# LouisPwr/CarpeDeam

Measured on AMD Instinct MI355X. Metric: corrected bases/sec on 50M×100bp synthetic reads (dhigh), 1/2/4/8 GPU, higher is better.
Workload: dtype u8 (2-bit packed bases; int32 scores; software x87 f80 likelihood sums)

## Files before the change

carpedeam_amd/csrc/bucket.h:

```cpp
#pragma once
#include <algorithm>
#include <cstdio>
#include <cstdlib>
#include <cstring>
#include <vector>

#include "common.h"
#include "radix.h"
#include "scan.h"

namespace bucket {

constexpr int BK_NT = 256;
constexpr int BK_WAVES = BK_NT / 64;
constexpr int WV_OWN = 256;
constexpr int WV_WIN = 768;
constexpr int WV_WORDS = WV_WIN / 64;
constexpr int WV_FIRST = 512;
constexpr int BK_GROUP = 256;
constexpr int BK_MAXB = 512;
constexpr int BK_ORD = 8;

__device__ __forceinline__ void waveLdsSync() {
    __builtin_amdgcn_fence(__ATOMIC_RELEASE, "wavefront");
    __builtin_amdgcn_wave_barrier();
    __builtin_amdgcn_fence(__ATOMIC_ACQUIRE, "wavefront");
}

template <int WIN> struct WaveLdsT {
    unsigned long long bits[WIN / 64];
    uint16_t ord[WIN];
};
typedef WaveLdsT<WV_WIN> WaveLds;
template <typename WL> __device__ __forceinline__ int firstSetFrom(const WL &w, int from, int limit) {
    for (int word = from >> 6; word * 64 < limit; word++) {
        unsigned long long m = w.bits[word];
        if (word == (from >> 6)) m &= ~0ull << (from & 63);
        if (m) { const int p = word * 64 + __ffsll(m) - 1; return p < limit ? p : -1; }
    }
    return -1;
}
template <typename WL> __device__ __forceinline__ int lastSetIn(const WL &w, int lo, int hi) {
    const int wl = (lo + 1) >> 6;
    for (int word = hi >> 6; word >= wl; word--) {
        unsigned long long m = w.bits[word];
        if (word == (hi >> 6)) m &= (2ull << (hi & 63)) - 1ull;
        if (word == wl) m &= ~0ull << ((lo + 1) & 63);
        if (m) return word * 64 + 63 - __clzll(m);
    }
    return -1;
}

struct BigList {
    unsigned long long *list;
    unsigned int *cnt;
    __device__ __forceinline__ void add(uint64_t s, uint64_t e) const { if (!list) return; const unsigned int q = atomicAdd(cnt, 1u); list[2 * (size_t) q] = s; list[2 * (size_t) q + 1] = e; }
};

template <int M> __device__ __forceinline__ uint32_t xorLane32(uint32_t a) {
    static_assert(M == 1 || M == 2 || M == 4 || M == 8 || M == 16 || M == 32, "lane distance");
    if (M == 1) return (uint32_t) __builtin_amdgcn_update_dpp(0, (int) a, 0xB1, 0xF, 0xF, false);
    if (M == 2) return (uint32_t) __builtin_amdgcn_update_dpp(0, (int) a, 0x4E, 0xF, 0xF, false);
    if (M == 4) {
        const int t = __builtin_amdgcn_update_dpp(0, (int) a, 0x104, 0xF, 0x5, false);
        return (uint32_t) __builtin_amdgcn_update_dpp(t, (int) a, 0x114, 0xF, 0xA, false);
    }
    if (M == 8) return (uint32_t) __builtin_amdgcn_update_dpp(0, (int) a, 0x128, 0xF, 0xF, false);
    if (M == 16) return (uint32_t) __builtin_amdgcn_ds_swizzle((int) a, 0x401F);
    return (uint32_t) __shfl_xor((int) a, 32, 64);
}
template <typename W, int M> struct XorLane;
template <int M> struct XorLane<uint32_t, M> { __device__ static __forceinline__ uint32_t get(uint32_t a) { return xorLane32<M>(a); } };
template <int M> struct XorLane<uint64_t, M> {
    __device__ static __forceinline__ uint64_t get(uint64_t a) { return ((uint64_t) xorLane32<M>((uint32_t) (a >> 32)) << 32) | xorLane32<M>((uint32_t) a); }
};
typedef unsigned __int128 u128;
template <int M> struct XorLane<u128, M> {
    __device__ static __forceinline__ u128 get(u128 a) { return ((u128) XorLane<uint64_t, M>::get((uint64_t) (a >> 64)) << 64) | XorLane<uint64_t, M>::get((uint64_t) a); }
};
template <typename W> __device__ __forceinline__ W xorLane(W a, int d) {
    switch (d) {
        case 1: return XorLane<W, 1>::get(a);
        case 2: return XorLane<W, 2>::get(a);
        case 4: return XorLane<W, 4>::get(a);
        case 8: return XorLane<W, 8>::get(a);
        case 16: return XorLane<W, 16>::get(a);
        default: return XorLane<W, 32>::get(a);
    }
}
template <typename W> __device__ __forceinline__ W shflUpW(W a, int d);
template <> __device__ __forceinline__ uint32_t shflUpW<uint32_t>(uint32_t a, int d) { return (uint32_t) __shfl_up((int) a, d, 64); }
template <> __device__ __forceinline__ uint64_t shflUpW<uint64_t>(uint64_t a, int d) {
    return ((uint64_t) (uint32_t) __shfl_up((int) (a >> 32), d, 64) << 32) | (uint32_t) __shfl_up((int) (uint32_t) a, d, 64);
}

template <int R, typename W>
__device__ __forceinline__ void bitonicRegs(W (&v)[R], int lane) {
#pragma unroll
    for (int k = 2; k <= 64 * R; k <<= 1) {
#pragma unroll
        for (int j = k >> 1; j > 0; j >>= 1) {
            if (j < R) {
#pragma unroll
                for (int r = 0; r < R; r++) {
                    const int p = r ^ j;
                    if (p > r) {
                        const bool up = (((lane * R + r) & k) == 0);
                        const W a = v[r], b = v[p];
                        const bool sw = (b < a) == up;
                        v[r] = sw ? b : a; v[p] = sw ? a : b;
                    }
                }
            } else {
                const bool lower = ((lane & (j / R)) == 0);
#pragma unroll
                for (int r = 0; r < R; r++) {
                    const bool up = (((lane * R + r) & k) == 0);
                    const W a = v[r], b = xorLane<W>(a, j / R);
                    v[r] = ((b < a) == (up == lower)) ? b : a;
                }
            }
        }
    }
}
template <int R, typename W, typename MakeComp, typename Done>
__device__ __forceinline__ void sortGroupRegs(int gm, int lane, const MakeComp &mk, const Done &done) {
    W v[R];
#pragma unroll
    for (int r = 0; r < R; r++) { const int i = lane * R + r; v[r] = (i < gm) ? mk(i) : (W) ~(W) 0; }
    bitonicRegs<R, W>(v, lane);
    done(v);
}
template <typename W, int MAXR = 8, typename MakeComp, typename Done>
__device__ __forceinline__ void sortGroup(int gm, int lane, const MakeComp &mk, const Done &done) {
    static_assert(MAXR == 1 || MAXR == 2 || MAXR == 4 || MAXR == 8, "networks of 64, 128, 256 and 512 words");
    if (MAXR == 1 || gm <= 64) sortGroupRegs<1, W>(gm, lane, mk, done);
    else if constexpr (MAXR >= 2) {
        if (MAXR == 2 || gm <= 128) sortGroupRegs<2, W>(gm, lane, mk, done);
        else if constexpr (MAXR >= 4) {
            if (MAXR == 4 || gm <= 256) sortGroupRegs<4, W>(gm, lane, mk, done);
            else if constexpr (MAXR >= 8) sortGroupRegs<8, W>(gm, lane, mk, done);
        }
    }
}
__device__ __forceinline__ uint64_t prevLane64(uint64_t a) {
    const uint32_t lo = (uint32_t) __builtin_amdgcn_update_dpp((int) (uint32_t) a, (int) (uint32_t) a, 0x138, 0xF, 0xF, false);
    const uint32_t hi = (uint32_t) __builtin_amdgcn_update_dpp((int) (uint32_t) (a >> 32), (int) (uint32_t) (a >> 32), 0x138, 0xF, 0xF, false);
    return ((uint64_t) hi << 32) | lo;
}
__device__ __forceinline__ uint64_t readLane64(uint64_t a, int l) {
    return ((uint64_t) (uint32_t) __builtin_amdgcn_readlane((int) (uint32_t) (a >> 32), l) << 32) | (uint32_t) __builtin_amdgcn_readlane((int) (uint32_t) a, l);
}

template <typename T, int WIN = WV_WIN, int FIRST = WV_FIRST, int GROUP = BK_GROUP, typename Fetch, typename Put, typename KeyAt, typename GroupFn>
__device__ __forceinline__ void waveBuckets(uint64_t r0, uint64_t n, int own, uint32_t maxBucket, uint64_t hiMask, const BigList &big, WaveLdsT<WIN> &w, int lane,
                                            const Fetch &fetch, const Put &put, const KeyAt &keyAt, const GroupFn &groupFn) {
    constexpr int WV_WIN = WIN, WV_FIRST = FIRST, WV_WORDS = WIN / 64;
    const int avail = (int) min((uint64_t) WV_WIN, n - r0);
    uint64_t carry = r0 ? keyAt(r0 - 1) : 0ull;
    int ordBase = -1;
    auto loadRows = [&](auto rowsTag, int t0, auto fullTag) {
        constexpr int ROWS = decltype(rowsTag)::value;
        constexpr bool FULL = decltype(fullTag)::value;
        T tup[ROWS];
#pragma unroll
        for (int t = 0; t < ROWS; t++) { const int i = (t0 + t) * 64 + lane; if (FULL || i < avail) tup[t] = fetch(r0 + (uint64_t) i); }
#pragma unroll
        for (int t = 0; t < ROWS; t++) {
            const int i = (t0 + t) * 64 + lane;
            const bool valid = FULL || i < avail;
            const uint64_t k = valid ? put(i, tup[t]) : 0ull;
            const bool differs = ((k ^ prevLane64(k)) & hiMask) != 0ull;
            unsigned long long m = __ballot(valid && differs) & ~1ull;
            if ((FULL || (t0 + t) * 64 < avail) && ((r0 == 0 && t0 + t == 0) || ((readLane64(k, 0) ^ carry) & hiMask) != 0ull)) m |= 1ull;
            if (lane == 0) w.bits[t0 + t] = m;
            const int below = (int) __builtin_amdgcn_mbcnt_hi((uint32_t) (m >> 32), __builtin_amdgcn_mbcnt_lo((uint32_t) m, 0u));
            if (valid) w.ord[i] = (uint16_t) (ordBase + below + (int) ((m >> lane) & 1ull));
            ordBase += __popcll(m);
            carry = readLane64(k, 63);
        }
    };
    if (lane >= WV_FIRST / 64 && lane < WV_WORDS) w.bits[lane] = 0ull;
    if (avail >= WV_FIRST) loadRows(std::integral_constant<int, WV_FIRST / 64>(), 0, std::true_type());
    else loadRows(std::integral_constant<int, WV_FIRST / 64>(), 0, std::false_type());
    waveLdsSync();
    const int ownEnd = min(own, avail);
    const int sLast = lastSetIn(w, -1, ownEnd - 1);
    if (sLast < 0) return;
    const int p0 = firstSetFrom(w, 0, ownEnd);
    int loaded = min(avail, WV_FIRST);
    int eLast = firstSetFrom(w, sLast + 1, loaded);
    if constexpr (WV_FIRST < WV_WIN) if (eLast < 0 && loaded < avail) {
        loadRows(std::integral_constant<int, WV_WORDS - WV_FIRST / 64>(), WV_FIRST / 64, std::false_type());
        waveLdsSync();
        loaded = avail;
        eLast = firstSetFrom(w, sLast + 1, loaded);
    }
    if (eLast < 0 && r0 + (uint64_t) avail == n) eLast = avail;
    int eOwn = eLast;
    if (eLast < 0) {
        const uint64_t h = keyAt(r0 + (uint64_t) sLast) & hiMask;
        uint64_t lo = r0 + (uint64_t) avail, hi = n;
        while (lo < hi) { const uint64_t mid = lo + ((hi - lo) >> 1); if ((keyAt(mid) & hiMask) == h) lo = mid + 1; else hi = mid; }
        if (lane == 0) big.add(r0 + (uint64_t) sLast, lo);
        eOwn = sLast;
    }
    int g0 = p0;
    while (g0 < eOwn) {
        const int lim = min(g0 + min(GROUP, (int) maxBucket), eOwn);
        int e = (lim == eOwn) ? eOwn : lastSetIn(w, g0, lim);
        if (e < 0) { e = firstSetFrom(w, g0 + 1, eOwn); if (e < 0) e = eOwn; }
        const int gm = e - g0;
        if (gm > (int) maxBucket) { if (lane == 0) big.add(r0 + (uint64_t) g0, r0 + (uint64_t) e); }
        else groupFn(g0, gm);
        g0 = e;
    }
}

constexpr int WV_IDX = 10;

struct SortArgs {
    const uint64_t *in; uint64_t *out; uint64_t n;
    int shiftHi;
    int ign;
    int own; uint32_t maxBucket;
    BigList big;
};

__global__ __launch_bounds__(BK_NT) void k_bucket_sort(SortArgs a) {
    __shared__ uint64_t sKeyAll[BK_WAVES][WV_WIN];
    __shared__ WaveLds wAll[BK_WAVES];
    const int lane = threadIdx.x & 63, wave = threadIdx.x >> 6;
    const uint64_t r0 = ((uint64_t) blockIdx.x * BK_WAVES + wave) * (uint64_t) a.own;
    if (r0 >= a.n) return;
    uint64_t *sKey = sKeyAll[wave];
    WaveLds &w = wAll[wave];
    const uint64_t lowMask = (1ull << a.shiftHi) - 1ull;
    const int lowW = a.shiftHi - a.ign, ign = a.ign;
    waveBuckets<uint64_t>(r0, a.n, a.own, a.maxBucket, ~lowMask, a.big, w, lane,
        [&](uint64_t g) { return a.in[g]; },
        [&](int i, uint64_t k) { sKey[i] = k; return k; },
        [&](uint64_t g) { return a.in[g]; },
        [&](int g0, int gm) {
            sortGroup<uint64_t>(gm, lane,
                [&](int i) {
                    const uint64_t low = (sKey[g0 + i] & lowMask) >> ign;
                    return ((((uint64_t) w.ord[g0 + i] << lowW) | low) << WV_IDX) | (uint64_t) (g0 + i);
                },
                [&](auto &v) {
                    constexpr int R = sizeof(v) / sizeof(v[0]);
#pragma unroll
                    for (int r = 0; r < R; r++) { const int p = lane * R + r; if (p < gm) a.out[r0 + (uint64_t) (g0 + p)] = sKey[(int) (v[r] & ((1u << WV_IDX) - 1u))]; }
                });
        });
}

template <int WAVES, typename W>
__device__ __forceinline__ void bitonicBlock(W (&v)[8], int lane, int wave, W *sX) {
    constexpr int R = 8, N = 64 * R * WAVES;
    const int base = wave * 64 * R + lane * R;
#pragma unroll
    for (int k = 2; k <= N; k <<= 1) {
#pragma unroll
        for (int j = k >> 1; j > 0; j >>= 1) {
            if (j >= 64 * R) {
                const int pw = wave ^ (j / (64 * R));
#pragma unroll
                for (int r = 0; r < R; r++) sX[(r * WAVES + wave) * 64 + lane] = v[r];
                __syncthreads();
                const bool lower = ((base & j) == 0);
#pragma unroll
                for (int r = 0; r < R; r++) {
                    const bool up = (((base + r) & k) == 0);
                    const W a = v[r], b = sX[(r * WAVES + pw) * 64 + lane];
                    v[r] = ((b < a) == (up == lower)) ? b : a;
                }
                __syncthreads();
            } else if (j >= R) {
                const bool lower = ((lane & (j / R)) == 0);
#pragma unroll
                for (int r = 0; r < R; r++) {
                    const bool up = (((base + r) & k) == 0);
                    const W a = v[r], b = xorLane<W>(a, j / R);
// ... 141 lines not shown
```

carpedeam_amd/csrc/kmer_group.h:

```cpp
#pragma once
#include "kmer_tuple.h"
#include "runsort.h"

namespace {

struct GroupParams {
    uint64_t n;
    int onlyExtendable, covMode; float covThr;
    uint32_t idBits, diagBits; int diagBias;
    int wide;
    uint64_t first;
    uint64_t firstRunIdx;
    unsigned long long *stat;
};
constexpr int STAT_STRIPES = 4096;
__device__ __forceinline__ void waveGroupStats(unsigned long long *stat, uint32_t cnt) {
    if ((threadIdx.x & 63) == 0 && cnt) atomicAdd(stat + ((blockIdx.x * 4 + (threadIdx.x >> 6)) & (STAT_STRIPES - 1)), (unsigned long long) cnt);
}
template <typename LY> struct GroupArgs : GroupParams {
    const uint64_t *keys; const typename LY::V *vals;
    TupleGeom geom;
};
__device__ __forceinline__ bool canBeCoveredK(float covThr, int covMode, float ql, float tl) {
    switch (covMode) {
        case 0: return ((ql / tl >= covThr) && (tl / ql >= covThr));
        case 2: return ((tl / ql) >= covThr);
        case 1: return ((ql / tl) >= covThr);
        case 3: return ((tl / ql) >= covThr) && (tl / ql) <= 1.0;
        case 4: return ((ql / tl) >= covThr) && (ql / tl) <= 1.0;
        case 5: return (fminf(tl, ql) / fmaxf(tl, ql)) >= covThr;
        default: return true;
    }
}
__device__ __forceinline__ uint64_t packGroupKey(const GroupParams &a, uint32_t rep, uint32_t id, int diag, bool noRev) {
    const uint64_t hi = a.wide ? (uint64_t) id : (((uint64_t) rep << a.idBits) | id);
    return (hi << (a.diagBits + 1)) | ((uint64_t) (uint32_t) (diag + a.diagBias) << 1) | (noRev ? 1ull : 0ull);
}
__device__ __forceinline__ uint64_t markRunStart(const GroupParams &a, uint64_t gk, uint32_t rep) {
    return (runsort::gkKept(gk) ? gk : (runsort::GK_DROPPED | ((uint64_t) rep << (a.diagBits + 1)))) | runsort::GK_START;
}
template <typename LY> struct StartIndex {
    const uint64_t *keys; TupleGeom geom; unsigned long long first;
    __device__ unsigned long long operator()(unsigned long long i) const {
        if (i == first) return i;
        const uint64_t a = keys[i], b = keys[i - 1];
        const bool start = (a == ~0ull) || (b == ~0ull) || (LY::kmerOf(a, i, geom) != LY::kmerOf(b, i - 1, geom));
        return start ? i : 0ull;
    }
};
template <typename LY> struct StartFrom {
    StartIndex<LY> f;
    __device__ __forceinline__ unsigned long long operator()(size_t i) const { return f(f.first + (unsigned long long) i); }
};

__device__ __forceinline__ uint64_t groupKeyCore(const GroupParams &a, uint32_t repId, int queryLen, int repPos, bool repIsReverse,
                                                 uint32_t id, int tLen, int tPos0, bool targetIsReverse) {
    int qPos, tPos; bool qRev;
    if (repIsReverse && !targetIsReverse) { qPos = repPos; tPos = tPos0; qRev = true; }
    else if (repIsReverse && targetIsReverse) { qPos = (queryLen - 1) - repPos; tPos = (tLen - 1) - tPos0; qRev = false; }
    else if (!repIsReverse && targetIsReverse) { qPos = (queryLen - 1) - repPos; tPos = (tLen - 1) - tPos0; qRev = true; }
    else { qPos = repPos; tPos = tPos0; qRev = false; }
    const int diagonal = qPos - tPos;
    const bool canBeExtended = diagonal < 0 || (diagonal > (queryLen - tLen));
    const bool cbc = (a.covThr <= 0.0f && a.covMode <= 2 && queryLen > 0 && tLen > 0) ? true : canBeCoveredK(a.covThr, a.covMode, (float) queryLen, (float) tLen);
    const bool keep = (a.onlyExtendable == 0 && cbc) || (canBeExtended && a.onlyExtendable != 0);
    return keep ? packGroupKey(a, repId, id, diagonal, !qRev) : ~0ull;
}
template <typename LY>
__device__ __forceinline__ uint64_t groupKeyOf(const GroupParams &a, const TupleGeom &geom, uint64_t repKey, typename LY::V repVal, uint64_t repSlot, uint32_t repPos0,
                                               bool firstRun, uint64_t key, typename LY::V v, uint64_t slot) {
    return groupKeyCore(a, LY::seqOf(repVal), (int) LY::lenOf(repKey, repVal, repSlot, geom), (int) repPos0, firstRun ? false : ((repKey & BIT63) == 0),
                        LY::seqOf(v), (int) LY::lenOf(key, v, slot, geom), (int) LY::posOf(key, v, slot, geom), (key & BIT63) == 0);
}

template <typename LY>
__global__ __launch_bounds__(256) void k_groups(GroupArgs<LY> a, unsigned long long *__restrict__ startIo ) {
    const uint64_t i = a.first + (uint64_t) blockIdx.x * blockDim.x + threadIdx.x;
    unsigned long long gk = ~0ull;
    if (i < a.n) {
        const uint64_t key = a.keys[i];
        if (key != ~0ull) {
            const uint64_t st = startIo[i];
            const uint64_t km = LY::kmerOf(key, i, a.geom);
            const bool hasNext = (i + 1 < a.n) && a.keys[i + 1] != ~0ull && LY::kmerOf(a.keys[i + 1], i + 1, a.geom) == km;
            if (st != i || hasNext) {
                uint64_t bestKey = a.keys[st]; const typename LY::V best = a.vals[st];
                const uint32_t repId = LY::seqOf(best);
                uint32_t bestPos = LY::posOf(bestKey, best, st, a.geom);
                for (uint64_t e = st + 1; e < a.n && a.keys[e] != ~0ull && LY::kmerOf(a.keys[e], e, a.geom) == km && LY::seqOf(a.vals[e]) == repId; e++) {
                    const uint32_t pe = LY::posOf(a.keys[e], a.vals[e], e, a.geom);
                    if (pe < bestPos) { bestPos = pe; bestKey = a.keys[e]; }
                }
                gk = groupKeyOf<LY>(a, a.geom, bestKey, best, st, bestPos, st == a.firstRunIdx, key, a.vals[i], i);
                if (a.wide && st == i) gk = markRunStart(a, gk, repId);
            }
        }
        startIo[i] = gk;
    }
    waveGroupStats(a.stat, (uint32_t) __popcll(__ballot(runsort::gkKept(gk))));
}

struct BlockHead { int32_t lo, hi; uint32_t td, pad; };
#ifndef CDM_REC_CAP
#define CDM_REC_CAP 32
#endif
constexpr int REC_CAP = CDM_REC_CAP;
static_assert(REC_CAP <= 64, "a wave writes its stage out with one lane per record");
__global__ void k_block_heads(TupleGeom geom, uint64_t n, uint64_t perBlock, uint64_t blocks, BlockHead *__restrict__ out) {
    const uint64_t b = (uint64_t) blockIdx.x * blockDim.x + threadIdx.x;
    if (b >= blocks) return;
    const uint64_t base = b * perBlock;
    const uint32_t td = headDigit(geom, base);
    const uint64_t since = base - geom.seg[td], until = geom.seg[td + 1] - base;
    BlockHead h; h.td = td; h.pad = 0; h.lo = -(int32_t) min(since, (uint64_t) 1 << 30); h.hi = (int32_t) min(until, (uint64_t) 1 << 30);
    out[b] = h;
}
constexpr int REC_WAVES = 256, REC_BIG_LDS = 256;
struct RecCount { const uint8_t *c; __device__ __forceinline__ unsigned long long operator()(size_t i) const { return c[i]; } };
__device__ __forceinline__ uint64_t lowerBoundStart(const uint64_t *__restrict__ val, uint64_t n, uint64_t start) {
    uint64_t lo = 0, hi = n;
    while (lo < hi) { const uint64_t mid = lo + ((hi - lo) >> 1); if ((val[mid] >> runsort::RUN_CNT_BITS) < start) lo = mid + 1; else hi = mid; }
    return lo;
}
__global__ __launch_bounds__(256) void k_rec_compact(const uint32_t *__restrict__ stRep, const uint64_t *__restrict__ stVal, const unsigned long long *__restrict__ off, uint64_t waves,
                                                     uint64_t own, const uint64_t *__restrict__ bigVal, uint64_t nBig, uint32_t *__restrict__ recRep, uint64_t *__restrict__ recVal) {
    __shared__ unsigned long long sOff[REC_WAVES + 1];
    __shared__ uint64_t sBig[REC_BIG_LDS];
    __shared__ uint64_t sB[2];
    const uint64_t w0 = (uint64_t) blockIdx.x * REC_WAVES;
    const int nw = (int) min((uint64_t) REC_WAVES, waves - w0);
    for (int i = threadIdx.x; i <= nw; i += 256) sOff[i] = off[w0 + i];
    if (threadIdx.x < 2) sB[threadIdx.x] = nBig ? lowerBoundStart(bigVal, nBig, (w0 + (threadIdx.x ? (uint64_t) nw : 0ull)) * own) : 0ull;
    __syncthreads();
    const uint64_t b0 = sB[0], nb = sB[1] - sB[0];
    for (uint64_t i = threadIdx.x; i < nb && i < (uint64_t) REC_BIG_LDS; i += 256) sBig[i] = bigVal[b0 + i] >> runsort::RUN_CNT_BITS;
    __syncthreads();
    const unsigned long long base = sOff[0], total = sOff[nw] - base;
    for (unsigned long long i = threadIdx.x; i < total; i += 256) {
        int w = 0;
#pragma unroll
        for (int st = REC_WAVES / 2; st > 0; st >>= 1) if (w + st < nw && sOff[w + st] - base <= i) w += st;
        const uint64_t src = (w0 + (uint64_t) w) * REC_CAP + (i - (sOff[w] - base));
        const uint64_t v = stVal[src], start = v >> runsort::RUN_CNT_BITS;
        uint64_t before = b0;
        if (nb <= (uint64_t) REC_BIG_LDS) { for (uint64_t q = 0; q < nb; q++) before += sBig[q] < start; }
        else before = lowerBoundStart(bigVal, nBig, start);
        recRep[base + i + before] = stRep[src]; recVal[base + i + before] = v;
    }
}
__global__ __launch_bounds__(256) void k_rec_place_big(const uint32_t *__restrict__ bigRep, const uint64_t *__restrict__ bigVal, uint64_t nBig, const uint64_t *__restrict__ stVal,
                                                       const uint8_t *__restrict__ stCnt, const unsigned long long *__restrict__ off, uint64_t own, uint32_t *__restrict__ recRep, uint64_t *__restrict__ recVal) {
    const uint64_t b = (uint64_t) blockIdx.x * blockDim.x + threadIdx.x;
    if (b >= nBig) return;
    const uint64_t v = bigVal[b], start = v >> runsort::RUN_CNT_BITS, w = start / own;
    uint64_t before = off[w];
    const int c = stCnt[w];
    for (int j = 0; j < c; j++) before += (stVal[w * REC_CAP + j] >> runsort::RUN_CNT_BITS) < start;
    recRep[b + before] = bigRep[b]; recVal[b + before] = v;
}
__global__ __launch_bounds__(256) void k_big_gap_copy(const unsigned long long *__restrict__ ranges, unsigned int cnt, const unsigned long long *__restrict__ dense, unsigned long long *__restrict__ gapped) {
    const unsigned int lane = threadIdx.x & 63, wavesPerGrid = gridDim.x * 4;
    for (unsigned int r = blockIdx.x * 4 + (threadIdx.x >> 6); r < cnt; r += wavesPerGrid) {
        const unsigned long long len = ranges[3 * (size_t) r + 1] - ranges[3 * (size_t) r], o = ranges[3 * (size_t) r + 2];
        for (unsigned long long i = lane; i < len; i += 64) gapped[o + r + i] = dense[o + i];
        if (lane == 0) gapped[o + r + len] = ~0ull;
    }
}
__global__ __launch_bounds__(256) void k_big_rec_starts(const unsigned long long *__restrict__ ranges, unsigned int cnt, uint64_t *__restrict__ recVal, uint64_t nRec) {
    const uint64_t j = (uint64_t) blockIdx.x * blockDim.x + threadIdx.x;
    if (j >= nRec) return;
    const uint64_t v = recVal[j], x = v >> runsort::RUN_CNT_BITS;
    unsigned int lo = 0, hi = cnt;
    while (hi - lo > 1) { const unsigned int mid = lo + ((hi - lo) >> 1); if (ranges[3 * (size_t) mid + 2] + mid <= x) lo = mid; else hi = mid; }
    const uint64_t slot = ranges[3 * (size_t) lo] + (x - (ranges[3 * (size_t) lo + 2] + lo));
    recVal[j] = (slot << runsort::RUN_CNT_BITS) | (v & ((1ull << runsort::RUN_CNT_BITS) - 1ull));
}
template <typename LY, typename W>
struct BucketGroupArgs : GroupParams {
    const BlockHead *blockHead = nullptr;
    uint32_t *recRep = nullptr; uint64_t *recVal = nullptr; uint8_t *recCnt = nullptr;
    uint32_t recLimit = REC_CAP;
    uint32_t *ovRep = nullptr; uint64_t *ovVal = nullptr; unsigned long long *ovCursor = nullptr; unsigned long long ovCap = 0;
    const uint64_t *keys; const typename LY::V *vals; TupleGeom geom;
    unsigned long long *out;
    int lowBits;
    int own; uint32_t maxBucket; bucket::BigList big;
};
#ifndef CDM_GK_OWN
#define CDM_GK_OWN 128
#define CDM_GK_WIN 384
#define CDM_GK_FIRST 256
#endif
#ifndef CDM_GKS_OWN
#define CDM_GKS_OWN 256
#define CDM_GKS_WIN 512
#define CDM_GKS_FIRST 384
#endif
#ifndef CDM_GKS_GROUP
#define CDM_GKS_GROUP 256
#endif
template <typename LY> struct GkGeom {
    static constexpr int OWN = LY::bySlot ? CDM_GKS_OWN : CDM_GK_OWN, WIN = LY::bySlot ? CDM_GKS_WIN : CDM_GK_WIN, FIRST = LY::bySlot ? CDM_GKS_FIRST : CDM_GK_FIRST, MAXB = WIN - OWN;
    static constexpr int GROUP = LY::bySlot ? CDM_GKS_GROUP : bucket::BK_GROUP, CAP = MAXB, MAXR = LY::bySlot ? CAP / 64 : 8;
    static_assert(WIN % 64 == 0 && FIRST % 64 == 0 && FIRST <= WIN && OWN <= FIRST && WIN <= (1 << bucket::WV_IDX) && (MAXB == 64 || MAXB == 128 || MAXB == 256 || MAXB == 512), "grouping kernel geometry");
    static_assert(GROUP >= 64 && GROUP <= MAXB && GROUP <= (1 << bucket::BK_ORD), "grouping kernel group capacity");
};
#ifndef CDM_GK_MINW
#define CDM_GK_MINW 0
#endif
template <typename LY> constexpr size_t gkLdsBytes() {
    return (size_t) bucket::BK_WAVES * ((size_t) GkGeom<LY>::WIN * 8 + (LY::bySlot ? 1 : (size_t) GkGeom<LY>::WIN) * sizeof(typename LY::V) + (size_t) GkGeom<LY>::CAP * 4 + sizeof(bucket::WaveLdsT<GkGeom<LY>::WIN>) +
                                      (LY::bySlot ? (size_t) REC_CAP : 1) * 12);
}
template <typename LY> constexpr int gkMinWaves() {
    return LY::bySlot ? (CDM_GK_MINW ? CDM_GK_MINW : 6) : (CDM_GK_MINW ? (int) std::min<size_t>(CDM_GK_MINW, CU_LDS_BYTES / gkLdsBytes<LY>()) : 1);
}
template <typename LY, typename W>
__global__ __launch_bounds__(bucket::BK_NT, gkMinWaves<LY>()) void k_bucket_groups(BucketGroupArgs<LY, W> a) {
    static_assert(bucket::BK_NT == 256 && (size_t) gkMinWaves<LY>() * gkLdsBytes<LY>() <= CU_LDS_BYTES, "the launch bound asks for more blocks per CU than the kernel's LDS lets run: the compiler would drop the request");
    using namespace bucket;
    typedef typename LY::V V;
    constexpr int GK_WIN = GkGeom<LY>::WIN, GK_FIRST = GkGeom<LY>::FIRST, GK_CAP = GkGeom<LY>::CAP;
    __shared__ uint64_t sKeyAll[BK_WAVES][GK_WIN];
    __shared__ V sValAll[BK_WAVES][LY::bySlot ? 1 : GK_WIN];
    __shared__ uint32_t sSAll[BK_WAVES][GK_CAP];
    static_assert(GK_CAP >= 64 * GkGeom<LY>::MAXR || !LY::bySlot, "the largest network of the instance writes 64 R words of sSAll");
    __shared__ WaveLdsT<GK_WIN> wAll[BK_WAVES];
    const int lane = threadIdx.x & 63, wave = threadIdx.x >> 6;
    const uint64_t r0 = ((uint64_t) blockIdx.x * BK_WAVES + wave) * (uint64_t) a.own;
    if (r0 >= a.n) return;
    uint64_t *sKey = sKeyAll[wave]; V *sVal = sValAll[wave]; uint32_t *ss = sSAll[wave];
    WaveLdsT<GK_WIN> &w = wAll[wave];
    const uint64_t hmask = (2ull << a.geom.kbits) - 1ull, lowMask = (1ull << a.lowBits) - 1ull;
    const int lowBits = a.lowBits;
    struct Tup { uint64_t k; V v; };
    constexpr uint32_t IDXM = (1u << WV_IDX) - 1u;
    uint32_t keptCnt = 0;
    uint32_t recCount = 0, prevRowKept = 0;
    constexpr bool REC = LY::bySlot;
    __shared__ uint32_t sRecRep[BK_WAVES][REC ? REC_CAP : 1];
    __shared__ uint64_t sRecVal[BK_WAVES][REC ? REC_CAP : 1];
    const uint32_t recLimit = a.recLimit;
    const uint64_t waveIdx = (uint64_t) blockIdx.x * BK_WAVES + wave;
    BlockHead bh; bh.lo = 0; bh.hi = 0; bh.td = 0; bh.pad = 0;
    const uint64_t blockBase = (uint64_t) blockIdx.x * BK_WAVES * (uint64_t) a.own;
    if constexpr (LY::bySlot) bh = a.blockHead[blockIdx.x];
    auto digitAt = [&](uint64_t g) -> uint32_t { const long long off = (long long) (g - blockBase); return (off >= (long long) bh.lo && off < (long long) bh.hi) ? bh.td : headDigit(a.geom, g); };
    waveBuckets<Tup, GK_WIN, GK_FIRST, GkGeom<LY>::GROUP>(r0, a.n, a.own, a.maxBucket, hmask & ~lowMask, a.big, w, lane,
        [&](uint64_t g) {
            Tup t;
            if constexpr (LY::bySlot) { t.k = a.keys[g]; t.v = digitAt(g); }
            else { t.k = a.keys[g]; t.v = a.vals[g]; }
            return t;
        },
        [&](int i, const Tup &t) {
            sKey[i] = t.k;
            if constexpr (LY::bySlot) return ((uint64_t) t.v << a.geom.headShift) | (t.k >> rx::SLOT_KEY_SHIFT);
            else { sVal[i] = t.v; return t.k; }
        },
        [&](uint64_t g) {
            if constexpr (LY::bySlot) return ((uint64_t) digitAt(g) << a.geom.headShift) | (a.keys[g] >> rx::SLOT_KEY_SHIFT);
            else return a.keys[g];
        },
        [&](int g0, int gm) {

            const int idxBits = (GK_CAP > 256 && gm > 256) ? 9 : 8, ord0 = w.ord[g0];
            sortGroup<W, GkGeom<LY>::MAXR>(gm, lane,
                [&](int i) {
                    const uint64_t low = LY::bySlot ? (uint64_t) ((uint32_t) (sKey[g0 + i] >> rx::SLOT_KEY_SHIFT)) & lowMask : sKey[g0 + i] & lowMask;
                    return (W) ((((W) (w.ord[g0 + i] - ord0) << lowBits | (W) low) << idxBits) | (W) i);
                },
                [&](auto &v) {
                    constexpr int R = sizeof(v) / sizeof(v[0]);
                    const W prevLast = shflUpW<W>(v[R - 1], 1);
                    int st[R], last = -1;
#pragma unroll
                    for (int r = 0; r < R; r++) {
                        const int p = lane * R + r;
                        const W prev = r ? v[r - 1] : prevLast;
                        if (p == 0 || (v[r] >> idxBits) != (prev >> idxBits)) last = p;
                        st[r] = last;
                    }
                    int sc = last;
#pragma unroll
                    for (int d = 1; d < 64; d <<= 1) { const int o = __shfl_up(sc, d, 64); if (lane >= d) sc = max(sc, o); }
                    const int carry = __shfl_up(sc, 1, 64);
#pragma unroll
                    for (int r = 0; r < R; r++) {
                        const int p = lane * R + r, s0 = st[r] < 0 ? carry : st[r];
                        ss[p] = (uint32_t) (g0 + (int) ((uint32_t) v[r] & ((1u << idxBits) - 1u))) | ((uint32_t) s0 << WV_IDX) | (s0 == p ? 1u << 31 : 0u);
                    }
                });
            waveLdsSync();
#pragma unroll 1
            for (int p = lane; p < gm; p += 64) {
                const uint32_t cw = ss[p];
                const int s0 = (int) ((cw >> WV_IDX) & 1023u), e = (int) (cw & IDXM), p0row = p - lane;
                unsigned long long gk = ~0ull;
                uint32_t recRepOfLane = 0;
                const bool hasNext = (p + 1 < gm) && !(ss[p + 1] >> 31);
                if constexpr (LY::bySlot) {
                if (s0 != p || hasNext) {
                    const int er = (int) (ss[s0] & IDXM);
                    uint32_t repId, bestPos, id, tPos; bool repFwd, fwd;
                    slotFields(a.geom, sKey[er], repId, bestPos, repFwd);
                    for (int t = s0 + 1; t < gm && !(ss[t] >> 31); t++) {
                        uint32_t ie, pe; bool fe;
                        slotFields(a.geom, sKey[(int) (ss[t] & IDXM)], ie, pe, fe);
                        if (ie != repId) break;
                        if (pe < bestPos) { bestPos = pe; repFwd = fe; }
                    }
                    slotFields(a.geom, sKey[e], id, tPos, fwd);
                    const bool firstRun = r0 + (uint64_t) (g0 + s0) == a.firstRunIdx;
                    gk = groupKeyCore(a, repId, (int) a.geom.uniL, (int) bestPos, firstRun ? false : !repFwd, id, (int) a.geom.uniL, (int) tPos, !fwd);
                    if (a.wide && s0 == p) gk = markRunStart(a, gk, repId);
                    recRepOfLane = repId;
                }
                } else
                if (s0 != p || hasNext) {
                    const int er = (int) (ss[s0] & IDXM);
                    uint64_t bestKey = sKey[er]; const V best = sVal[er];
                    const uint32_t repId = LY::seqOf(best);
                    uint32_t repLen, bestPos;
                    LY::unpackR1(bestKey, best, a.geom, repLen, bestPos);
                    for (int t = s0 + 1; t < gm && !(ss[t] >> 31); t++) {
                        const int et = (int) (ss[t] & IDXM);
                        if (LY::seqOf(sVal[et]) != repId) break;
                        uint32_t le, pe;
                        LY::unpackR1(sKey[et], sVal[et], a.geom, le, pe);
                        if (pe < bestPos) { bestPos = pe; bestKey = sKey[et]; }
                    }
                    const uint64_t key = sKey[e]; const V val = sVal[e];
                    uint32_t tLen, tPos;
                    LY::unpackR1(key, val, a.geom, tLen, tPos);
                    const bool firstRun = r0 + (uint64_t) (g0 + s0) == a.firstRunIdx;
                    gk = groupKeyCore(a, repId, (int) repLen, (int) bestPos, firstRun ? false : ((bestKey & BIT63) == 0), LY::seqOf(val), (int) tLen, (int) tPos, (key & BIT63) == 0);
                    if (a.wide && s0 == p) gk = markRunStart(a, gk, repId);
                    recRepOfLane = repId;
                }
                a.out[r0 + (uint64_t) (g0 + p)] = gk;
                const unsigned long long keptMask = __ballot(runsort::gkKept(gk));
                keptCnt += (uint32_t) __popcll(keptMask);
                if constexpr (REC) if (a.recRep) {
                    const uint32_t recBase = (uint32_t) __builtin_amdgcn_readfirstlane((int) recCount);
                    const bool lastKept = __builtin_amdgcn_readfirstlane((int) prevRowKept) != 0;
                    const unsigned long long startMask = __ballot((cw >> 31) != 0u);
                    const bool runsOn = p0row != 0 && lastKept && (keptMask & 1ull) && !(startMask & 1ull) && recBase - 1u < recLimit;
                    const unsigned long long begins = keptMask & (startMask | ~(keptMask << 1)) & ~(runsOn ? 1ull : 0ull), ends = ~keptMask | startMask;
                    if (((begins >> lane) & 1ull) || (runsOn && lane == 0)) {
                        const unsigned long long behind = lane == 63 ? 0ull : ends >> (lane + 1);
                        const uint32_t len = behind ? (uint32_t) __ffsll(behind) : (uint32_t) (64 - lane);
                        const uint32_t j = recBase + (uint32_t) __popcll(begins & ((1ull << lane) - 1ull));
                        const uint64_t rv = ((r0 + (uint64_t) (g0 + p)) << runsort::RUN_CNT_BITS) | (uint64_t) len;
                        if (runsOn && lane == 0) atomicAdd(reinterpret_cast<unsigned long long *>(&sRecVal[wave][recBase - 1u]), (unsigned long long) len);
                        else if (j < recLimit) { sRecRep[wave][j] = recRepOfLane; sRecVal[wave][j] = rv; }
                        else { const unsigned long long q = atomicAdd(a.ovCursor, 1ull); if (q < a.ovCap) { a.ovRep[q] = recRepOfLane; a.ovVal[q] = rv; } }
                    }
                    recCount = recBase + (uint32_t) __popcll(begins);
                    prevRowKept = (uint32_t) (keptMask >> 63);
                }
            }
            waveLdsSync();
        });
    waveGroupStats(a.stat, keptCnt);
    recCount = (uint32_t) __builtin_amdgcn_readfirstlane((int) recCount);
    if constexpr (REC) if (a.recRep && recCount) {
        const uint32_t m = min(recCount, recLimit);
        waveLdsSync();
        if ((uint32_t) lane < m) { const uint64_t slot = waveIdx * (uint64_t) REC_CAP + (uint32_t) lane; a.recRep[slot] = sRecRep[wave][lane]; a.recVal[slot] = sRecVal[wave][lane]; }
        if (lane == 0) a.recCnt[waveIdx] = (uint8_t) m;
    }
}

__global__ __launch_bounds__(256) void k_reduce_stats(const unsigned long long *__restrict__ stripes, unsigned long long *__restrict__ out) {
    unsigned long long c = 0;
    for (int i = threadIdx.x; i < STAT_STRIPES; i += 256) c += stripes[i];
    c = cdm_block_sum<unsigned long long>(c);
    if (threadIdx.x == 0) out[0] = c;
}
__global__ void k_live_count(const uint64_t *__restrict__ keys, uint64_t n, int kbits, unsigned long long *__restrict__ out) {
    uint64_t lo = 0, hi = n;
    while (lo < hi) { const uint64_t mid = lo + ((hi - lo) >> 1); if ((keys[mid] >> kbits) & 1ull) hi = mid; else lo = mid + 1; }
    *out = lo;
}
__global__ void k_count_hash_tuples(const uint64_t *__restrict__ keys, uint64_t n, unsigned long long *__restrict__ out) {
    uint64_t lo = 0, hi = n;
    while (lo < hi) { const uint64_t mid = lo + ((hi - lo) >> 1); if (keys[mid] == ~0ull) hi = mid; else lo = mid + 1; }
    *out = lo;
}
constexpr int STALE_MAX = CDM_STALE_MAX;
constexpr int STALE_BUCKET = 2048;
template <typename LY>
struct StaleArgs {
    const uint64_t *keys; const typename LY::V *vals; TupleGeom geom;
    uint64_t live, kmerSlots, nTuples, J; int lowBits; bool sorted;
    uint32_t *out;
};
template <typename LY>
__global__ __launch_bounds__(256) void k_stale_tail(StaleArgs<LY> a) {
    __shared__ uint64_t sC[STALE_BUCKET];
    __shared__ uint64_t sB[2];
    __shared__ int sSel;
    const uint64_t hmask = (2ull << a.geom.kbits) - 1ull, lowMask = (1ull << a.lowBits) - 1ull;
    uint32_t cnt = 0, target = ~0u;
    for (uint64_t j = a.J; cnt < (uint32_t) STALE_MAX; j++) {
        uint64_t idx;
        if (j < a.live) {
            idx = j;
            if (!a.sorted) {
                if (threadIdx.x == 0) {
                    const uint64_t h = (memSortBits<LY>(a.keys, j, a.geom) & hmask) >> a.lowBits;
                    uint64_t lo = 0, hi = j;
                    while (lo < hi) { const uint64_t mid = lo + ((hi - lo) >> 1); if (((memSortBits<LY>(a.keys, mid, a.geom) & hmask) >> a.lowBits) < h) lo = mid + 1; else hi = mid; }
                    sB[0] = lo;
                    lo = j; hi = a.live;
                    while (lo < hi) { const uint64_t mid = lo + ((hi - lo) >> 1); if (((memSortBits<LY>(a.keys, mid, a.geom) & hmask) >> a.lowBits) == h) lo = mid + 1; else hi = mid; }
                    sB[1] = lo;
                }
                __syncthreads();
                const uint64_t b0 = sB[0], b1 = sB[1];
                const int m = (int) min((uint64_t) STALE_BUCKET + 1, b1 - b0);
                if (m <= STALE_BUCKET) {
                    for (int i = threadIdx.x; i < m; i += blockDim.x) sC[i] = ((memSortBits<LY>(a.keys, b0 + i, a.geom) & lowMask) << 12) | (uint64_t) i;
                    if (threadIdx.x == 0) sSel = 0;
                    __syncthreads();
                    const int want = (int) (j - b0);
                    for (int e = threadIdx.x; e < m; e += blockDim.x) {
                        const uint64_t mine = sC[e]; int r = 0;
                        for (int f = 0; f < m; f++) r += sC[f] < mine;
                        if (r == want) sSel = e;
                    }
                    __syncthreads();
                    idx = b0 + (uint64_t) sSel;
                }
                __syncthreads();
            }
        } else {
            idx = a.kmerSlots + (j - a.live);
            if (idx >= a.nTuples) break;
        }
        if (a.keys[idx] == ~0ull) break;
        uint64_t key; typename LY::V v;
        memPair<LY>(a.keys, a.vals, idx, a.geom, key, v);
        if (cnt == 0) target = LY::seqOf(v);
        else if (LY::seqOf(v) != target) break;
        if (threadIdx.x == 0) a.out[2 + cnt] = LY::posOf(key, v, idx, a.geom);
        cnt++;
    }
    if (threadIdx.x == 0) { a.out[0] = cnt; a.out[1] = target; }
}
__global__ void k_first_diff(const uint64_t *__restrict__ a, const uint64_t *__restrict__ b, uint64_t n, unsigned long long *__restrict__ out) {
    for (uint64_t i = (uint64_t) blockIdx.x * blockDim.x + threadIdx.x; i < n; i += (uint64_t) gridDim.x * blockDim.x)
        if (a[i] != b[i]) { atomicMin(out, (unsigned long long) i); return; }
}
template <bool GATHER>
__global__ __launch_bounds__(256) void k_big_slot_pairs(const unsigned long long *__restrict__ ranges, unsigned int cnt, uint64_t *arr, TupleGeom geom, uint64_t *denseK, uint32_t *denseV) {
    const unsigned int lane = threadIdx.x & 63, wavesPerGrid = gridDim.x * 4;
    for (unsigned int r = blockIdx.x * 4 + (threadIdx.x >> 6); r < cnt; r += wavesPerGrid) {
        const unsigned long long s = ranges[3 * (size_t) r], e = ranges[3 * (size_t) r + 1], o = ranges[3 * (size_t) r + 2];
        const uint32_t td = headDigit(geom, s);
        for (unsigned long long i = lane; i < e - s; i += 64) {
            if (GATHER) { uint64_t key; uint32_t id; slotTupleToPair(geom, arr[s + i], td, key, id); denseK[o + i] = key; denseV[o + i] = id; }
            else arr[s + i] = pairToSlotTuple(geom, denseK[o + i], denseV[o + i]);
        }
    }
}

}
```

carpedeam_amd/csrc/kmer_tuple.h:

```cpp
#pragma once
#include "radix.h"

namespace {

constexpr uint64_t BIT63 = 1ull << 63;
__host__ __device__ __forceinline__ uint64_t rotl64(uint64_t x, int r) { return (x << r) | (x >> (64 - r)); }
__host__ __device__ __forceinline__ uint64_t xxh64_u64(uint64_t in, uint64_t seed) {
    const uint64_t P1 = 11400714785074694791ULL, P2 = 14029467366897019727ULL, P3 = 1609587929392839161ULL, P4 = 9650029242287828579ULL,
                   P5 = 2870177450012600261ULL;
    uint64_t h = seed + P5 + 8;
    uint64_t k1 = in * P2; k1 = rotl64(k1, 31); k1 *= P1;
    h ^= k1; h = rotl64(h, 27) * P1 + P4;
    h ^= h >> 33; h *= P2; h ^= h >> 29; h *= P3; h ^= h >> 32;
    return h;
}
__device__ __forceinline__ uint64_t revComplement(uint64_t kmer, int k) {
    uint64_t x = kmer ^ 0xAAAAAAAAAAAAAAAAULL;
    x = ((x >> 2) & 0x3333333333333333ULL) | ((x & 0x3333333333333333ULL) << 2);
    x = ((x >> 4) & 0x0F0F0F0F0F0F0F0FULL) | ((x & 0x0F0F0F0F0F0F0F0FULL) << 4);
    x = __builtin_bswap64(x);
    return x >> (64 - 2 * k);
}

struct TupleGeom {
    int kbits, lb;
    uint64_t kmerSlots;
    const uint32_t *lenArr;
    uint32_t uniS = 0, uniL = 0; int uniK = 0; uint32_t uniMul = 0; int uniSh = 0;
    const unsigned long long *seg = nullptr; int headShift = 0;
};
inline void divMagic(uint32_t d, uint32_t &mul, int &sh) {
    int l = 0; while ((1ull << l) < d) l++;
    mul = (uint32_t) ((((1ull << l) - d) << 32) / d + 1ull); sh = l > 0 ? l - 1 : 0;
    if (d == 1) { mul = 0; sh = 0; }
}
__device__ __forceinline__ uint32_t headDigit(const TupleGeom &g, uint64_t idx) {
    uint32_t d = 0;
#pragma unroll
    for (uint32_t st = rx::BINS / 2; st > 0; st >>= 1) if (g.seg[d + st] <= idx) d += st;
    return d;
}
__device__ __forceinline__ uint32_t headDigitUniform(const TupleGeom &g, uint64_t idx) {
    const uint64_t u = ((uint64_t) (uint32_t) __builtin_amdgcn_readfirstlane((int) (uint32_t) (idx >> 32)) << 32) | (uint32_t) __builtin_amdgcn_readfirstlane((int) (uint32_t) idx);
    uint32_t d = 0;
#pragma unroll
    for (uint32_t st = rx::BINS / 2; st > 0; st >>= 1) { const unsigned long long b = g.seg[d + st]; if (b <= u) d += st; }
    return (uint32_t) __builtin_amdgcn_readfirstlane((int) d);
}
__device__ __forceinline__ void slotSplit(const TupleGeom &g, uint32_t slot, uint32_t &seq, uint32_t &r) {
    const uint32_t t = __umulhi(slot, g.uniMul);
    const uint32_t q = g.uniS == 1u ? slot : (t + ((slot - t) >> 1)) >> g.uniSh;
    seq = q; r = slot - q * g.uniS;
}
template <int FB>
struct LayoutWideT {
    typedef uint64_t V;
    static constexpr bool bySlot = false;
    static constexpr uint64_t FM = (1ull << FB) - 1ull;
    __device__ static void store(uint64_t *keys, V *vals, uint64_t slot, uint64_t kmer63, bool fwd, uint32_t seq, uint32_t L, uint32_t pos, const TupleGeom &) {
        keys[slot] = kmer63 | (fwd ? BIT63 : 0ull); vals[slot] = ((uint64_t) seq << (2 * FB)) | ((uint64_t) L << FB) | pos;
    }
    __device__ static void storeHash(uint64_t *keys, V *vals, uint64_t slot, uint64_t hash64, uint32_t seq, uint32_t L, const TupleGeom &) {
        keys[slot] = hash64; vals[slot] = ((uint64_t) seq << (2 * FB)) | ((uint64_t) L << FB);
    }
    __device__ static void storeEmpty(uint64_t *keys, V *vals, uint64_t slot) { keys[slot] = ~0ull; vals[slot] = 0; }
    __device__ static uint64_t kmerOf(uint64_t key, uint64_t, const TupleGeom &) { return key & ~BIT63; }
    __device__ static uint32_t seqOf(V v) { return (uint32_t) (v >> (2 * FB)); }
    __device__ static uint32_t lenOf(uint64_t, V v, uint64_t, const TupleGeom &) { return (uint32_t) ((v >> FB) & FM); }
    __device__ static uint32_t posOf(uint64_t, V v, uint64_t, const TupleGeom &) { return (uint32_t) (v & FM); }
    __device__ static void unpackR1(uint64_t, V v, const TupleGeom &, uint32_t &len, uint32_t &pos) { pos = (uint32_t) (v & FM); len = (uint32_t) ((v >> FB) & FM); }
};
typedef LayoutWideT<16> LayoutWide;
typedef LayoutWideT<20> LayoutLong;
struct LayoutHuge {
    typedef uint64_t V;
    static constexpr bool bySlot = false;
    __device__ static void store(uint64_t *keys, V *vals, uint64_t slot, uint64_t kmer63, bool fwd, uint32_t seq, uint32_t, uint32_t pos, const TupleGeom &) {
        keys[slot] = kmer63 | (fwd ? BIT63 : 0ull); vals[slot] = ((uint64_t) seq << 32) | pos;
    }
    __device__ static void storeHash(uint64_t *keys, V *vals, uint64_t slot, uint64_t hash64, uint32_t seq, uint32_t, const TupleGeom &) { keys[slot] = hash64; vals[slot] = (uint64_t) seq << 32; }
    __device__ static void storeEmpty(uint64_t *keys, V *vals, uint64_t slot) { keys[slot] = ~0ull; vals[slot] = 0; }
    __device__ static uint64_t kmerOf(uint64_t key, uint64_t, const TupleGeom &) { return key & ~BIT63; }
    __device__ static uint32_t seqOf(V v) { return (uint32_t) (v >> 32); }
    __device__ static uint32_t lenOf(uint64_t, V v, uint64_t, const TupleGeom &g) { return g.lenArr[(uint32_t) (v >> 32)]; }
    __device__ static uint32_t posOf(uint64_t, V v, uint64_t, const TupleGeom &) { return (uint32_t) v; }
    __device__ static void unpackR1(uint64_t, V v, const TupleGeom &g, uint32_t &len, uint32_t &pos) { pos = (uint32_t) v; len = g.lenArr[(uint32_t) (v >> 32)]; }
};
struct LayoutPacked {
    typedef uint32_t V;
    static constexpr bool bySlot = false;
    __device__ static void store(uint64_t *keys, V *vals, uint64_t slot, uint64_t kmer63, bool fwd, uint32_t seq, uint32_t L, uint32_t pos, const TupleGeom &g) {
        keys[slot] = kmer63 | ((uint64_t) pos << (g.kbits + 1)) | ((uint64_t) L << (g.kbits + 1 + g.lb)) | (fwd ? BIT63 : 0ull); vals[slot] = seq;
    }
    __device__ static void storeHash(uint64_t *keys, V *vals, uint64_t slot, uint64_t hash64, uint32_t seq, uint32_t L, const TupleGeom &g) {
        keys[slot] = (slot < g.kmerSlots) ? (hash64 | ((uint64_t) L << (g.kbits + 1 + g.lb))) : hash64; vals[slot] = seq;
    }
    __device__ static void storeEmpty(uint64_t *keys, V *vals, uint64_t slot) { keys[slot] = ~0ull; vals[slot] = 0; }
    __device__ static uint64_t kmerOf(uint64_t key, uint64_t slot, const TupleGeom &g) { return slot < g.kmerSlots ? (key & ((1ull << g.kbits) - 1ull)) : (key & ~BIT63); }
    __device__ static uint32_t seqOf(V v) { return v; }
    __device__ static uint32_t lenOf(uint64_t key, V v, uint64_t slot, const TupleGeom &g) { return slot < g.kmerSlots ? (uint32_t) ((key >> (g.kbits + 1 + g.lb)) & ((1ull << g.lb) - 1ull)) : g.lenArr[v]; }
    __device__ static uint32_t posOf(uint64_t key, V, uint64_t slot, const TupleGeom &g) { return slot < g.kmerSlots ? (uint32_t) ((key >> (g.kbits + 1)) & ((1ull << g.lb) - 1ull)) : 0u; }
    __device__ static void unpackR1(uint64_t key, V, const TupleGeom &g, uint32_t &len, uint32_t &pos) {
        const uint32_t t = (uint32_t) (key >> (g.kbits + 1)), m = (1u << g.lb) - 1u;
        pos = t & m; len = (t >> g.lb) & m;
    }
};
struct LayoutSlot {
    typedef uint32_t V;
    static constexpr bool bySlot = true;
    __device__ static void store(uint64_t *keys, V *, uint64_t slot, uint64_t kmer63, bool fwd, uint32_t, uint32_t, uint32_t, const TupleGeom &) { keys[slot] = kmer63 | (fwd ? BIT63 : 0ull); }
    __device__ static void storeHash(uint64_t *keys, V *vals, uint64_t slot, uint64_t hash64, uint32_t seq, uint32_t, const TupleGeom &g) { keys[slot] = hash64; if (slot >= g.kmerSlots) vals[slot] = seq; }
    __device__ static void storeEmpty(uint64_t *keys, V *, uint64_t slot) { keys[slot] = ~0ull; }
    __device__ static uint64_t kmerOf(uint64_t key, uint64_t slot, const TupleGeom &g) { return LayoutPacked::kmerOf(key, slot, g); }
    __device__ static uint32_t seqOf(V v) { return v; }
    __device__ static uint32_t lenOf(uint64_t key, V v, uint64_t slot, const TupleGeom &g) { return LayoutPacked::lenOf(key, v, slot, g); }
    __device__ static uint32_t posOf(uint64_t key, V v, uint64_t slot, const TupleGeom &g) { return LayoutPacked::posOf(key, v, slot, g); }
    __device__ static void unpackR1(uint64_t key, V v, const TupleGeom &g, uint32_t &len, uint32_t &pos) { LayoutPacked::unpackR1(key, v, g, len, pos); }
};
__device__ __forceinline__ void slotFields(const TupleGeom &g, uint64_t t8, uint32_t &id, uint32_t &pos, bool &fwd) {
    fwd = ((uint32_t) (t8 >> rx::SLOT_STRAND_SHIFT) & 1u) != 0u;
    uint32_t r;
    slotSplit(g, (uint32_t) t8, id, r);
    pos = r == 0u ? 0u : (fwd ? r - 1u : g.uniL - (r - 1u) - (uint32_t) g.uniK);
}
__device__ __forceinline__ void slotTupleToPair(const TupleGeom &g, uint64_t t8, uint32_t td, uint64_t &key, uint32_t &id) {
    static_assert(rx::SLOT_STRAND_SHIFT == 32 && rx::SLOT_KEY_SHIFT == 33, "the tuple's high word is k-mer bits << 1 | strand");
    const uint32_t hiw = (uint32_t) (t8 >> 32);
    const bool fwd = (hiw & 1u) != 0u;
    uint32_t r;
    slotSplit(g, (uint32_t) t8, id, r);
    const uint32_t pos = r == 0u ? 0u : (fwd ? r - 1u : g.uniL - (r - 1u) - (uint32_t) g.uniK);
    if (g.kbits + 1 >= 32) {
        const uint32_t lo = (hiw >> 1) | (td << g.headShift);
        const uint32_t hi = (g.headShift ? td >> (32 - g.headShift) : 0u) | (pos << (g.kbits + 1 - 32)) | (g.uniL << (g.kbits + 1 + g.lb - 32)) | (fwd ? 0x80000000u : 0u);
        key = ((uint64_t) hi << 32) | lo;
    } else {
        const uint64_t kmer = ((uint64_t) td << g.headShift) | (uint64_t) (hiw >> 1);
        key = kmer | ((uint64_t) pos << (g.kbits + 1)) | ((uint64_t) g.uniL << (g.kbits + 1 + g.lb)) | (fwd ? BIT63 : 0ull);
    }
}
__device__ __forceinline__ uint64_t pairToSlotTuple(const TupleGeom &g, uint64_t key, uint32_t id) {
    uint32_t len, pos;
    LayoutPacked::unpackR1(key, id, g, len, pos);
    const bool fwd = (key & BIT63) != 0ull;
    const uint32_t slot = id * g.uniS + 1u + (fwd ? pos : g.uniL - pos - (uint32_t) g.uniK);
    return ((key & ((1ull << g.headShift) - 1ull)) << rx::SLOT_KEY_SHIFT) | ((fwd ? 1ull : 0ull) << rx::SLOT_STRAND_SHIFT) | (uint64_t) slot;
}
template <typename LY> __device__ __forceinline__ uint64_t memSortBits(const uint64_t *keys, uint64_t idx, const TupleGeom &g) {
    if constexpr (LY::bySlot) { if (idx < g.kmerSlots) return ((uint64_t) headDigit(g, idx) << g.headShift) | (keys[idx] >> rx::SLOT_KEY_SHIFT); }
    return keys[idx] & ((2ull << g.kbits) - 1ull);
}
template <typename LY> __device__ __forceinline__ void memPair(const uint64_t *keys, const typename LY::V *vals, uint64_t idx, const TupleGeom &g, uint64_t &key, typename LY::V &v) {
    if constexpr (LY::bySlot) { if (idx < g.kmerSlots) { uint32_t id; slotTupleToPair(g, keys[idx], headDigit(g, idx), key, id); v = id; return; } }
    key = keys[idx]; v = vals[idx];
}

}
```

Before: 19.64 billion.

## Specialize 32-bit bitonic sort with DPP moves and streamline group-key computation

Adds a compile-time bitonic network for 32-bit words that uses DPP and ds_swizzle lane moves plus min/max in place of generic xor shuffles and compare-swaps. It also simplifies the diagonal computation in groupKeyCore, makes the wave index uniform via readfirstlane, and skips the best-position scan when the next slot cannot belong to the same read. First-run and output indexing are precomputed per wave as 32-bit offsets. The mirror-based network and the early-exit slot test add correctness risk if the lane patterns or range checks are off.

```diff
diff --git a/carpedeam_amd/csrc/bucket.h b/carpedeam_amd/csrc/bucket.h
--- a/carpedeam_amd/csrc/bucket.h
+++ b/carpedeam_amd/csrc/bucket.h
@@ -3,6 +3,7 @@
 #include <cstdio>
 #include <cstdlib>
 #include <cstring>
+#include <type_traits>
 #include <vector>
 
 #include "common.h"
@@ -123,12 +124,69 @@
         }
     }
 }
+template <int CTRL> __device__ __forceinline__ uint32_t dppMove(uint32_t a) {
+    return (uint32_t) __builtin_amdgcn_update_dpp(0, (int) a, CTRL, 0xF, 0xF, true);
+}
+template <int M> __device__ __forceinline__ uint32_t mirrorLane32(uint32_t a) {
+    static_assert(M == 1 || M == 3 || M == 7 || M == 15 || M == 31 || M == 63, "mirror image inside 2, 4 .. 64 lanes");
+    if (M == 1) return dppMove<0xB1>(a);
+    if (M == 3) return dppMove<0x1B>(a);
+    if (M == 7) return dppMove<0x141>(a);
+    if (M == 15) return dppMove<0x140>(a);
+    if (M == 31) return (uint32_t) __builtin_amdgcn_ds_swizzle((int) a, 0x7C1F);
+    return (uint32_t) __shfl_xor((int) a, 63, 64);
+}
+template <int M> __device__ __forceinline__ uint32_t xorLaneFold32(uint32_t a) {
+    static_assert(M == 1 || M == 2 || M == 4 || M == 8 || M == 16, "lane distance");
+    if (M == 1) return dppMove<0xB1>(a);
+    if (M == 2) return dppMove<0x4E>(a);
+    if (M == 4) return dppMove<0x1B>(dppMove<0x141>(a));
+    if (M == 8) return dppMove<0x128>(a);
+    return (uint32_t) __builtin_amdgcn_ds_swizzle((int) a, 0x401F);
+}
+template <int R> __device__ __forceinline__ void keepLowerOrUpper(uint32_t (&v)[R], const uint32_t (&b)[R], bool lower) {
+    uint32_t lo[R], hi[R];
+#pragma unroll
+    for (int r = 0; r < R; r++) { lo[r] = min(v[r], b[r]); hi[r] = max(v[r], b[r]); }
+#pragma unroll
+    for (int r = 0; r < R; r++) v[r] = lower ? lo[r] : hi[r];
+}
+template <int R, int J> __device__ __forceinline__ void bitonicStage32(uint32_t (&v)[R], int lane) {
+    if constexpr (J < R) {
+#pragma unroll
+        for (int r = 0; r < R; r++) if ((r ^ J) > r) { const uint32_t a = v[r], b = v[r ^ J]; v[r] = min(a, b); v[r ^ J] = max(a, b); }
+    } else {
+        uint32_t b[R];
+#pragma unroll
+        for (int r = 0; r < R; r++) b[r] = xorLaneFold32<J / R>(v[r]);
+        keepLowerOrUpper<R>(v, b, (lane & (J / R)) == 0);
+    }
+}
+template <int R, int K> __device__ __forceinline__ void bitonicMirror32(uint32_t (&v)[R], int lane) {
+    if constexpr (K <= R) {
+#pragma unroll
+        for (int r = 0; r < R; r++) if ((r ^ (K - 1)) > r) { const uint32_t a = v[r], b = v[r ^ (K - 1)]; v[r] = min(a, b); v[r ^ (K - 1)] = max(a, b); }
+    } else {
+        uint32_t b[R];
+#pragma unroll
+        for (int r = 0; r < R; r++) b[r] = mirrorLane32<K / R - 1>(v[R - 1 - r]);
+        keepLowerOrUpper<R>(v, b, (lane & (K / (2 * R))) == 0);
+    }
+}
+template <int R, int K, int J> __device__ __forceinline__ void bitonicMerge32(uint32_t (&v)[R], int lane) {
+    if constexpr (J > 0) { bitonicStage32<R, J>(v, lane); bitonicMerge32<R, K, (J >> 1)>(v, lane); }
+}
+template <int R, int K> __device__ __forceinline__ void bitonicLevels32(uint32_t (&v)[R], int lane) {
+    if constexpr (K <= 64 * R) { bitonicMirror32<R, K>(v, lane); bitonicMerge32<R, K, (K >> 2)>(v, lane); bitonicLevels32<R, 2 * K>(v, lane); }
+}
+template <int R>
+__device__ __forceinline__ void bitonicRegs32(uint32_t (&v)[R], int lane) { bitonicLevels32<R, 2>(v, lane); }
 template <int R, typename W, typename MakeComp, typename Done>
 __device__ __forceinline__ void sortGroupRegs(int gm, int lane, const MakeComp &mk, const Done &done) {
     W v[R];
 #pragma unroll
     for (int r = 0; r < R; r++) { const int i = lane * R + r; v[r] = (i < gm) ? mk(i) : (W) ~(W) 0; }
-    bitonicRegs<R, W>(v, lane);
+    if constexpr (std::is_same<W, uint32_t>::value) bitonicRegs32<R>(v, lane); else bitonicRegs<R, W>(v, lane);
     done(v);
 }
 template <typename W, int MAXR = 8, typename MakeComp, typename Done>
diff --git a/carpedeam_amd/csrc/kmer_group.h b/carpedeam_amd/csrc/kmer_group.h
--- a/carpedeam_amd/csrc/kmer_group.h
+++ b/carpedeam_amd/csrc/kmer_group.h
@@ -55,12 +55,9 @@
 
 __device__ __forceinline__ uint64_t groupKeyCore(const GroupParams &a, uint32_t repId, int queryLen, int repPos, bool repIsReverse,
                                                  uint32_t id, int tLen, int tPos0, bool targetIsReverse) {
-    int qPos, tPos; bool qRev;
-    if (repIsReverse && !targetIsReverse) { qPos = repPos; tPos = tPos0; qRev = true; }
-    else if (repIsReverse && targetIsReverse) { qPos = (queryLen - 1) - repPos; tPos = (tLen - 1) - tPos0; qRev = false; }
-    else if (!repIsReverse && targetIsReverse) { qPos = (queryLen - 1) - repPos; tPos = (tLen - 1) - tPos0; qRev = true; }
-    else { qPos = repPos; tPos = tPos0; qRev = false; }
-    const int diagonal = qPos - tPos;
+    const bool qRev = repIsReverse != targetIsReverse;
+    const int plain = repPos - tPos0;
+    const int diagonal = targetIsReverse ? (queryLen - tLen) - plain : plain;
     const bool canBeExtended = diagonal < 0 || (diagonal > (queryLen - tLen));
     const bool cbc = (a.covThr <= 0.0f && a.covMode <= 2 && queryLen > 0 && tLen > 0) ? true : canBeCoveredK(a.covThr, a.covMode, (float) queryLen, (float) tLen);
     const bool keep = (a.onlyExtendable == 0 && cbc) || (canBeExtended && a.onlyExtendable != 0);
@@ -226,7 +223,7 @@
     __shared__ uint32_t sSAll[BK_WAVES][GK_CAP];
     static_assert(GK_CAP >= 64 * GkGeom<LY>::MAXR || !LY::bySlot, "the largest network of the instance writes 64 R words of sSAll");
     __shared__ WaveLdsT<GK_WIN> wAll[BK_WAVES];
-    const int lane = threadIdx.x & 63, wave = threadIdx.x >> 6;
+    const int lane = threadIdx.x & 63, wave = LY::bySlot ? __builtin_amdgcn_readfirstlane((int) (threadIdx.x >> 6)) : (int) (threadIdx.x >> 6);
     const uint64_t r0 = ((uint64_t) blockIdx.x * BK_WAVES + wave) * (uint64_t) a.own;
     if (r0 >= a.n) return;
     uint64_t *sKey = sKeyAll[wave]; V *sVal = sValAll[wave]; uint32_t *ss = sSAll[wave];
@@ -241,6 +238,8 @@
     __shared__ uint32_t sRecRep[BK_WAVES][REC ? REC_CAP : 1];
     __shared__ uint64_t sRecVal[BK_WAVES][REC ? REC_CAP : 1];
     const uint32_t recLimit = a.recLimit;
+    const uint32_t firstRel = a.firstRunIdx - r0 < (uint64_t) GK_WIN ? (uint32_t) (a.firstRunIdx - r0) : ~0u;
+    unsigned long long *const outW = a.out + r0;
     const uint64_t waveIdx = (uint64_t) blockIdx.x * BK_WAVES + wave;
     BlockHead bh; bh.lo = 0; bh.hi = 0; bh.td = 0; bh.pad = 0;
     const uint64_t blockBase = (uint64_t) blockIdx.x * BK_WAVES * (uint64_t) a.own;
@@ -302,16 +301,20 @@
                 if constexpr (LY::bySlot) {
                 if (s0 != p || hasNext) {
                     const int er = (int) (ss[s0] & IDXM);
-                    uint32_t repId, bestPos, id, tPos; bool repFwd, fwd;
-                    slotFields(a.geom, sKey[er], repId, bestPos, repFwd);
-                    for (int t = s0 + 1; t < gm && !(ss[t] >> 31); t++) {
-                        uint32_t ie, pe; bool fe;
-                        slotFields(a.geom, sKey[(int) (ss[t] & IDXM)], ie, pe, fe);
-                        if (ie != repId) break;
-                        if (pe < bestPos) { bestPos = pe; repFwd = fe; }
+                    uint32_t repId, bestPos, id, tPos, repR; bool repFwd, fwd;
+                    const uint64_t repT = sKey[er];
+                    slotFields(a.geom, repT, repId, bestPos, repFwd, repR);
+                    const uint32_t nextSlot = (uint32_t) sKey[(int) (ss[s0 + 1] & IDXM)];
+                    if (nextSlot - (uint32_t) repT < a.geom.uniS - repR) {
+                        for (int t = s0 + 1; t < gm && !(ss[t] >> 31); t++) {
+                            uint32_t ie, pe; bool fe;
+                            slotFields(a.geom, sKey[(int) (ss[t] & IDXM)], ie, pe, fe);
+                            if (ie != repId) break;
+                            if (pe < bestPos) { bestPos = pe; repFwd = fe; }
+                        }
                     }
                     slotFields(a.geom, sKey[e], id, tPos, fwd);
-                    const bool firstRun = r0 + (uint64_t) (g0 + s0) == a.firstRunIdx;
+                    const bool firstRun = (uint32_t) (g0 + s0) == firstRel;
                     gk = groupKeyCore(a, repId, (int) a.geom.uniL, (int) bestPos, firstRun ? false : !repFwd, id, (int) a.geom.uniL, (int) tPos, !fwd);
                     if (a.wide && s0 == p) gk = markRunStart(a, gk, repId);
                     recRepOfLane = repId;
@@ -338,7 +341,8 @@
                     if (a.wide && s0 == p) gk = markRunStart(a, gk, repId);
                     recRepOfLane = repId;
                 }
-                a.out[r0 + (uint64_t) (g0 + p)] = gk;
+                if constexpr (LY::bySlot) outW[(uint32_t) (g0 + p)] = gk;
+                else a.out[r0 + (uint64_t) (g0 + p)] = gk;
                 const unsigned long long keptMask = __ballot(runsort::gkKept(gk));
                 keptCnt += (uint32_t) __popcll(keptMask);
                 if constexpr (REC) if (a.recRep) {
diff --git a/carpedeam_amd/csrc/kmer_tuple.h b/carpedeam_amd/csrc/kmer_tuple.h
--- a/carpedeam_amd/csrc/kmer_tuple.h
+++ b/carpedeam_amd/csrc/kmer_tuple.h
@@ -117,11 +117,16 @@
     __device__ static uint32_t posOf(uint64_t key, V v, uint64_t slot, const TupleGeom &g) { return LayoutPacked::posOf(key, v, slot, g); }
     __device__ static void unpackR1(uint64_t key, V v, const TupleGeom &g, uint32_t &len, uint32_t &pos) { LayoutPacked::unpackR1(key, v, g, len, pos); }
 };
+__device__ __forceinline__ void slotFields(const TupleGeom &g, uint64_t t8, uint32_t &id, uint32_t &pos, bool &fwd, uint32_t &r) {
+    fwd = ((uint32_t) (t8 >> rx::SLOT_STRAND_SHIFT) & 1u) != 0u;
+    slotSplit(g, (uint32_t) t8, id, r);
+    const uint32_t pf = r - 1u, pr = (g.uniL + 1u - (uint32_t) g.uniK) - r;
+    const uint32_t p = fwd ? pf : pr;
+    pos = r == 0u ? 0u : p;
+}
 __device__ __forceinline__ void slotFields(const TupleGeom &g, uint64_t t8, uint32_t &id, uint32_t &pos, bool &fwd) {
-    fwd = ((uint32_t) (t8 >> rx::SLOT_STRAND_SHIFT) & 1u) != 0u;
     uint32_t r;
-    slotSplit(g, (uint32_t) t8, id, r);
-    pos = r == 0u ? 0u : (fwd ? r - 1u : g.uniL - (r - 1u) - (uint32_t) g.uniK);
+    slotFields(g, t8, id, pos, fwd, r);
 }
 __device__ __forceinline__ void slotTupleToPair(const TupleGeom &g, uint64_t t8, uint32_t td, uint64_t &key, uint32_t &id) {
     static_assert(rx::SLOT_STRAND_SHIFT == 32 && rx::SLOT_KEY_SHIFT == 33, "the tuple's high word is k-mer bits << 1 | strand");
```

Result: faster. 20.35 billion, median of 6 (+3.6%).
